# sunnyHelen/JPerceiver

Hardware: AMD Instinct MI355X
Metric: train images/sec (full train step, synthetic 3-frame batches) (higher is better)
Workload: dtype f32

## Files before the change

jperceiver_amd/csrc/conv_c16.hip:

```cpp
#include "jp_common.h"
#include <algorithm>

namespace {

constexpr int TPB = 256;

template <int CI, int CO, bool UPIN, bool SUMOUT, bool TRANS>
__global__ __launch_bounds__(TPB) void c16_conv_kernel(const float* __restrict__ x, const float* __restrict__ w,
                                                       const float* __restrict__ bias, float* __restrict__ y, int H, int W, int act,
                                                       int accumulate) {
    __shared__ __attribute__((aligned(16))) float wl[CI * 9 * CO];
    for (int i = threadIdx.x; i < CI * 9 * CO; i += TPB) {
        const int co = i % CO, tap = (i / CO) % 9, ci = i / (9 * CO);
        wl[i] = TRANS ? w[((size_t)ci * CO + co) * 9 + (8 - tap)] : w[((size_t)co * CI + ci) * 9 + tap];
    }
    __syncthreads();
    const int img = blockIdx.z;
    const int y0 = blockIdx.y * 32 + (threadIdx.x >> 4) * 2, x0 = blockIdx.x * 32 + (threadIdx.x & 15) * 2;
    const int sh = UPIN ? 1 : 0, hs = H >> sh, ws = W >> sh;
    const float* xp = x + (size_t)img * CI * hs * ws;
    int off[4][4];
#pragma unroll
    for (int a = 0; a < 4; ++a)
#pragma unroll
// ... 57 lines not shown
    }
}

constexpr int WG_R = 4, WG_C = 64;
template <int CI, int CO, bool UPIN, bool PART>
__global__ __launch_bounds__(TPB) void c16_wgrad_kernel(const float* __restrict__ x, const float* __restrict__ dy, float* __restrict__ dw,
                                                        int H, int W, int ntiles) {
    constexpr int P = CI * CO / TPB;
    static_assert(CI * CO % TPB == 0, "pairs per thread");
    constexpr int DP = WG_C + 1, XP = WG_C + 3;
    __shared__ float dT[CO * WG_R * DP];
    __shared__ float xT[CI * (WG_R + 2) * XP];
    const int sh = UPIN ? 1 : 0, hs = H >> sh, ws = W >> sh;
    const int tiles_x = W / WG_C, tiles_img = tiles_x * (H / WG_R);
    float acc[P][9];
#pragma unroll
    for (int k = 0; k < P; ++k)
#pragma unroll
        for (int t = 0; t < 9; ++t) acc[k][t] = 0.f;
    for (int T = blockIdx.x; T < ntiles; T += gridDim.x) {
        const int img = T / tiles_img, r_ = T - img * tiles_img;
        const int y0 = (r_ / tiles_x) * WG_R, x0 = (r_ % tiles_x) * WG_C;
        __syncthreads();
        const float* dp = dy + (size_t)img * CO * H * W;
        for (int i = threadIdx.x; i < CO * WG_R * WG_C; i += TPB) {
            const int c = i % WG_C, r = (i / WG_C) % WG_R, co = i / (WG_C * WG_R);
            dT[(co * WG_R + r) * DP + c] = dp[((size_t)co * H + y0 + r) * W + x0 + c];
        }
        const float* xp = x + (size_t)img * CI * hs * ws;
        for (int i = threadIdx.x; i < CI * (WG_R + 2) * (WG_C + 2); i += TPB) {
            const int c = i % (WG_C + 2), r = (i / (WG_C + 2)) % (WG_R + 2), ci = i / ((WG_C + 2) * (WG_R + 2));
            const int yy = y0 - 1 + r, xx = x0 - 1 + c;
            const bool in = (unsigned)yy < (unsigned)H && (unsigned)xx < (unsigned)W;
            xT[(ci * (WG_R + 2) + r) * XP + c] = in ? xp[((size_t)ci * hs + (yy >> sh)) * ws + (xx >> sh)] : 0.f;
        }
        __syncthreads();
#pragma unroll
        for (int k = 0; k < P; ++k) {
            const int q = threadIdx.x + TPB * k, co = q / CI, ci = q - co * CI;
            const float* dr = dT + co * WG_R * DP;
            const float* xr = xT + ci * (WG_R + 2) * XP;
#pragma unroll 1
            for (int r = 0; r < WG_R; ++r) {
                float w0[3], w1[3], w2[3];
#pragma unroll
                for (int t = 0; t < 3; ++t) {
                    w0[t] = xr[(r + t) * XP + 0];
                    w1[t] = xr[(r + t) * XP + 1];
                }
#pragma unroll 4
                for (int c = 0; c < WG_C; ++c) {
#pragma unroll
                    for (int t = 0; t < 3; ++t) w2[t] = xr[(r + t) * XP + c + 2];
                    const float d = dr[r * DP + c];
#pragma unroll
                    for (int t = 0; t < 3; ++t) {
                        acc[k][3 * t + 0] = fmaf(d, w0[t], acc[k][3 * t + 0]);
                        acc[k][3 * t + 1] = fmaf(d, w1[t], acc[k][3 * t + 1]);
                        acc[k][3 * t + 2] = fmaf(d, w2[t], acc[k][3 * t + 2]);
                    }
#pragma unroll
                    for (int t = 0; t < 3; ++t) { w0[t] = w1[t]; w1[t] = w2[t]; }
                }
            }
        }
    }
#pragma unroll
    for (int k = 0; k < P; ++k) {
        const int q = threadIdx.x + TPB * k;
#pragma unroll
        for (int t = 0; t < 9; ++t) {
            if (PART) dw[(size_t)blockIdx.x * (CO * CI * 9) + (size_t)q * 9 + t] = acc[k][t];
            else atomicAdd(dw + (size_t)q * 9 + t, acc[k][t]);
        }
    }
}

__global__ void c16_wgrad_fold_kernel(const float* __restrict__ part, float* __restrict__ dw, int n, int nblocks) {
    const int i = blockIdx.x * blockDim.x + threadIdx.x;
    if (i >= n) return;
    float s = 0.f;
    for (int b = 0; b < nblocks; ++b) s += part[(size_t)b * n + i];
    dw[i] += s;
}

template <bool UPIN, bool SUMOUT, bool TRANS>
int launch_conv(const float* x, const float* w, const float* bias, float* y, int N, int CI, int CO, int H, int W, int act, int accumulate,
                hipStream_t st) {
    const dim3 grid(W / 32, H / 32, N);
#define JP_GO(A, B)                                                                                                          \
    hipLaunchKernelGGL((c16_conv_kernel<A, B, UPIN, SUMOUT, TRANS>), grid, dim3(TPB), 0, st, x, w, bias, y, H, W, act, accumulate)
    if (CI == 16 && CO == 16) JP_GO(16, 16);
    else if (CI == 32 && CO == 32) JP_GO(32, 32);
    else if (CI == 32 && CO == 16) JP_GO(32, 16);
    else if (CI == 16 && CO == 32) JP_GO(16, 32);
    else return 1;
#undef JP_GO
    return 0;
}

}

bool jp_c16_ok(int Cin, int Cout, int KH, int stride, int pad, int pad_mode, int H, int W) {
    static const bool on = [] { const char* e = getenv("JP_C16"); return !(e && e[0] == '0'); }();
    return on && Cin == 16 && Cout == 16 && KH == 3 && stride == 1 && pad == 1 && pad_mode == 0 &&
           H % 32 == 0 && W % 64 == 0 && H >= 64;
}
int jp_c16_fwd(const float* x, int up, const float* w, const float* bias, float* y, int N, int Cin, int Cout, int H, int W, int act,
               hipStream_t st) {
    return up ? launch_conv<true, false, false>(x, w, bias, y, N, Cin, Cout, H, W, act, 0, st)
              : launch_conv<false, false, false>(x, w, bias, y, N, Cin, Cout, H, W, act, 0, st);
}
int jp_c16_dgrad(const float* dy, const float* w, float* dx, int up, int N, int Cin, int Cout, int H, int W, int accumulate,
                 hipStream_t st) {
    return up ? launch_conv<false, true, true>(dy, w, nullptr, dx, N, Cout, Cin, H, W, 0, accumulate, st)
              : launch_conv<false, false, true>(dy, w, nullptr, dx, N, Cout, Cin, H, W, 0, accumulate, st);
}
long jp_c16_wgrad_ws_floats(int N, int Cin, int Cout, int H, int W) {
    return (long)std::min(N * (H / WG_R) * (W / WG_C), 512) * Cout * Cin * 9;
}
int jp_c16_wgrad(const float* x, int up, const float* dy, float* dw, int N, int Cin, int Cout, int H, int W, hipStream_t st,
                 float* ws, long ws_floats) {
    const int ntiles = N * (H / WG_R) * (W / WG_C);
    const dim3 grid(std::min(ntiles, 512));
    const int nw = Cout * Cin * 9;
    const bool part = ws && ws_floats >= (long)grid.x * nw;
    float* out = part ? ws : dw;
#define JP_GO1(A, B, U, P) hipLaunchKernelGGL((c16_wgrad_kernel<A, B, U, P>), grid, dim3(TPB), 0, st, x, dy, out, H, W, ntiles)
#define JP_GO(A, B)                                                                     \
    {                                                                                   \
        if (up) { if (part) JP_GO1(A, B, true, true); else JP_GO1(A, B, true, false); } \
        else { if (part) JP_GO1(A, B, false, true); else JP_GO1(A, B, false, false); }  \
    }
    if (Cin == 16 && Cout == 16) JP_GO(16, 16)
    else if (Cin == 32 && Cout == 32) JP_GO(32, 32)
    else if (Cin == 32 && Cout == 16) JP_GO(32, 16)
    else if (Cin == 16 && Cout == 32) JP_GO(16, 32)
    else return 1;
#undef JP_GO
#undef JP_GO1
    if (part) hipLaunchKernelGGL(c16_wgrad_fold_kernel, dim3((nw + 255) / 256), dim3(256), 0, st, ws, dw, nw, (int)grid.x);
    return 0;
}
```

jperceiver_amd/csrc/conv_small.hip:

```cpp
#include "jp_common.h"
#include <algorithm>

namespace {

constexpr int TPB = 256;
constexpr int MAXCO = 4;

struct SrcSeg {
    const float* p;
    int C, sh;
};
struct Src3s {
    SrcSeg s[3];
    int nseg, H, W;
};

__device__ __forceinline__ void tap_offsets(int y, int x, int H, int W, int sh, int reflect, int off[9]) {
    const int w = W >> sh;
#pragma unroll
    for (int t = 0; t < 9; ++t) {
        int iy = y - 1 + t / 3, ix = x - 1 + t % 3;
        if (reflect) {
            iy = jp_reflect(iy, H);
            ix = jp_reflect(ix, W);
// ... 130 lines not shown
            }
            __syncthreads();
            const int xo = tx0 + tx;
            float g[4][CO];
#pragma unroll
            for (int j = 0; j < 4; ++j) {
                const int yo = ty0 + q * 4 + j;
                const bool ok = yo < H && xo < W;
#pragma unroll
                for (int c = 0; c < CO; ++c) g[j][c] = ok ? dp[(size_t)c * HW + yo * W + xo] : 0.f;
            }
#pragma unroll
            for (int r = 0; r < 6; ++r) {
                const float* row = tile + (q * 4 + r) * PW + tx;
                const float v0 = row[0], v1 = row[1], v2 = row[2];
#pragma unroll
                for (int j = 0; j < 4; ++j) {
                    const int ky = r - j;
                    if (ky < 0 || ky > 2) continue;
#pragma unroll
                    for (int c = 0; c < CO; ++c) {
                        acc[c * 9 + ky * 3 + 0] = fmaf(g[j][c], v0, acc[c * 9 + ky * 3 + 0]);
                        acc[c * 9 + ky * 3 + 1] = fmaf(g[j][c], v1, acc[c * 9 + ky * 3 + 1]);
                        acc[c * 9 + ky * 3 + 2] = fmaf(g[j][c], v2, acc[c * 9 + ky * 3 + 2]);
                    }
                }
            }
        }
    }
    const int lane = threadIdx.x & 63, wv = threadIdx.x >> 6;
#pragma unroll
    for (int i = 0; i < CO * 9; ++i) {
        const float s = jp_wave_sum(acc[i]);
        if (lane == 0) red[wv][i] = s;
    }
    __syncthreads();
    if (threadIdx.x < CO * 9) {
        const int i = threadIdx.x;
        const float s = red[0][i] + red[1][i] + red[2][i] + red[3][i];
        const int c = i / 9, t = i - c * 9;
        if (part) part[(((size_t)blockIdx.z * gridDim.x + blockIdx.x) * Cin + ci) * (CO * 9) + i] = s;
        else atomicAdd(dw + ((size_t)c * Cin + ci) * 9 + t, s);
    }
}

__global__ void conv_small_wgrad_fold_kernel(const float* __restrict__ part, float* __restrict__ dw, int Cin, int CO, int nwg) {
    const int i = blockIdx.x * blockDim.x + threadIdx.x;
    if (i >= Cin * CO * 9) return;
    const int ci = i / (CO * 9), r = i - ci * (CO * 9), c = r / 9, t = r - c * 9;
    float s = 0.f;
    for (int b = 0; b < nwg; ++b) s += part[((size_t)b * Cin + ci) * (CO * 9) + r];
    dw[((size_t)c * Cin + ci) * 9 + t] += s;
}

Src3s make_src(const float* x0, int c0, int up0, const float* x1, int c1, int up1, const float* x2, int c2, int up2,
               int H, int W) {
    Src3s s;
    s.nseg = 0;
    s.H = H; s.W = W;
    const float* ps[3] = {x0, x1, x2};
    const int cs[3] = {c0, c1, c2}, us[3] = {up0, up1, up2};
    for (int i = 0; i < 3; ++i)
        if (cs[i] > 0) { s.s[s.nseg].p = ps[i]; s.s[s.nseg].C = cs[i]; s.s[s.nseg].sh = us[i]; ++s.nseg; }
    for (int i = s.nseg; i < 3; ++i) s.s[i] = s.s[0];
    return s;
}

__device__ __forceinline__ void up_tap_range(int a, int r, int& lo, int& hi) {
    lo = a ? (r ? 2 : 0) : (r ? 1 : 0);
    hi = a ? (r ? 2 : 1) : (r ? 2 : 0);
}
__device__ __forceinline__ void up_build_weights(const float* __restrict__ w, float* wq, int C) {
    for (int i = threadIdx.x; i < 16 * C; i += blockDim.x) {
        const int c = i % C, q = i / C;
        int y0, y1, x0, x1;
        up_tap_range(q >> 3, (q >> 1) & 1, y0, y1);
        up_tap_range((q >> 2) & 1, q & 1, x0, x1);
        float v = 0.f;
        for (int dy = y0; dy <= y1; ++dy)
            for (int dx = x0; dx <= x1; ++dx) v += w[c * 9 + dy * 3 + dx];
        wq[i] = v;
    }
}
__device__ __forceinline__ void up_gather_D(const float* __restrict__ dyp, int i, int j, int h, int w, float D[16]) {
    const int W = 2 * w;
#pragma unroll
    for (int q = 0; q < 16; ++q) {
        const int a = q >> 3, b = (q >> 2) & 1, r = (q >> 1) & 1, s = q & 1;
        const int ri = i + 1 - a - r, rj = j + 1 - b - s;
        const int ei = (i == 0 && a == 0 && r == 0) ? 0 : ((i == h - 1 && a == 1 && r == 1) ? h - 1 : -1);
        const int ej = (j == 0 && b == 0 && s == 0) ? 0 : ((j == w - 1 && b == 1 && s == 1) ? w - 1 : -1);
        const bool rv = (unsigned)ri < (unsigned)h, cv = (unsigned)rj < (unsigned)w;
        float v = 0.f;
        if (rv && cv) v += dyp[(2 * ri + a) * W + 2 * rj + b];
        if (ei >= 0 && cv) v += dyp[(2 * ei + a) * W + 2 * rj + b];
        if (rv && ej >= 0) v += dyp[(2 * ri + a) * W + 2 * ej + b];
        if (ei >= 0 && ej >= 0) v += dyp[(2 * ei + a) * W + 2 * ej + b];
        D[q] = v;
    }
}

__global__ __launch_bounds__(TPB) void up_head_fwd_kernel(const float* __restrict__ x, const float* __restrict__ w,
                                                          const float* __restrict__ bias, float* __restrict__ y, int C,
                                                          int h, int wd, int act) {
    extern __shared__ float wq[];
    up_build_weights(w, wq, C);
    __syncthreads();
    const int img = blockIdx.y, hw = h * wd;
    const int p = blockIdx.x * TPB + threadIdx.x;
    if (p >= hw) return;
    const int i = p / wd, j = p - i * wd;
    const int r0 = max(i - 1, 0) * wd, r1 = i * wd, r2 = min(i + 1, h - 1) * wd;
    const int c0 = max(j - 1, 0), c2 = min(j + 1, wd - 1);
    float o00 = 0.f, o01 = 0.f, o10 = 0.f, o11 = 0.f;
    const float* xp = x + (size_t)img * C * hw;
    for (int c = 0; c < C; ++c) {
        const float* q = xp + (size_t)c * hw;
        const float v00 = q[r0 + c0], v01 = q[r0 + j], v02 = q[r0 + c2];
        const float v10 = q[r1 + c0], v11 = q[r1 + j], v12 = q[r1 + c2];
        const float v20 = q[r2 + c0], v21 = q[r2 + j], v22 = q[r2 + c2];
        const float* wc = wq + c;
        o00 += wc[0 * C] * v00 + wc[1 * C] * v01 + wc[2 * C] * v10 + wc[3 * C] * v11;
        o01 += wc[4 * C] * v01 + wc[5 * C] * v02 + wc[6 * C] * v11 + wc[7 * C] * v12;
        o10 += wc[8 * C] * v10 + wc[9 * C] * v11 + wc[10 * C] * v20 + wc[11 * C] * v21;
        o11 += wc[12 * C] * v11 + wc[13 * C] * v12 + wc[14 * C] * v21 + wc[15 * C] * v22;
    }
    const float bv = bias ? bias[0] : 0.f;
    float* yo = y + (size_t)img * 4 * hw + (size_t)(2 * i) * (2 * wd) + 2 * j;
    *reinterpret_cast<float2*>(yo) = make_float2(jp_act(o00 + bv, act), jp_act(o01 + bv, act));
    *reinterpret_cast<float2*>(yo + 2 * wd) = make_float2(jp_act(o10 + bv, act), jp_act(o11 + bv, act));
}

__global__ __launch_bounds__(TPB) void up_head_fwd2_kernel(const float* __restrict__ x, const float* __restrict__ w,
                                                           const float* __restrict__ bias, float* __restrict__ y, int C,
                                                           int h, int wd, int act) {
    extern __shared__ float wq[];
    up_build_weights(w, wq, C);
    __syncthreads();
    const int img = blockIdx.y, hw = h * wd, w2 = wd >> 1;
    const int p = blockIdx.x * TPB + threadIdx.x;
    if (p >= h * w2) return;
    const int i = p / w2, j = 2 * (p - i * w2);
    const int r0 = max(i - 1, 0) * wd, r1 = i * wd, r2 = min(i + 1, h - 1) * wd;
    const int cl = max(j - 1, 0), cr = min(j + 2, wd - 1);
    float o[2][4];
#pragma unroll
    for (int k = 0; k < 2; ++k)
#pragma unroll
        for (int q = 0; q < 4; ++q) o[k][q] = 0.f;
    const float* xp = x + (size_t)img * C * hw;
#pragma unroll 4
    for (int c = 0; c < C; ++c) {
        const float* q = xp + (size_t)c * hw;
        float v[3][4];
        const int rr[3] = {r0, r1, r2};
#pragma unroll
        for (int r = 0; r < 3; ++r) {
            const float2 m = *reinterpret_cast<const float2*>(q + rr[r] + j);
            v[r][0] = q[rr[r] + cl]; v[r][1] = m.x; v[r][2] = m.y; v[r][3] = q[rr[r] + cr];
        }
        float wc[16];
#pragma unroll
        for (int t = 0; t < 16; ++t) wc[t] = wq[t * C + c];
#pragma unroll
        for (int k = 0; k < 2; ++k) {
            o[k][0] += wc[0] * v[0][k] + wc[1] * v[0][k + 1] + wc[2] * v[1][k] + wc[3] * v[1][k + 1];
            o[k][1] += wc[4] * v[0][k + 1] + wc[5] * v[0][k + 2] + wc[6] * v[1][k + 1] + wc[7] * v[1][k + 2];
            o[k][2] += wc[8] * v[1][k] + wc[9] * v[1][k + 1] + wc[10] * v[2][k] + wc[11] * v[2][k + 1];
            o[k][3] += wc[12] * v[1][k + 1] + wc[13] * v[1][k + 2] + wc[14] * v[2][k + 1] + wc[15] * v[2][k + 2];
        }
    }
    const float bv = bias ? bias[0] : 0.f;
    float* yo = y + (size_t)img * 4 * hw + (size_t)(2 * i) * (2 * wd) + 2 * j;
    *reinterpret_cast<float4*>(yo) = make_float4(jp_act(o[0][0] + bv, act), jp_act(o[0][1] + bv, act), jp_act(o[1][0] + bv, act),
                                                 jp_act(o[1][1] + bv, act));
    *reinterpret_cast<float4*>(yo + 2 * wd) = make_float4(jp_act(o[0][2] + bv, act), jp_act(o[0][3] + bv, act),
                                                          jp_act(o[1][2] + bv, act), jp_act(o[1][3] + bv, act));
}

template <int groups>
__global__ __launch_bounds__(TPB) void up_head_fwd2s_kernel(const float* __restrict__ x, const float* __restrict__ w,
                                                           const float* __restrict__ bias, float* __restrict__ y, int C,
                                                           int h, int wd, int act) {
    extern __shared__ float wq[];
    __shared__ float red[3][64][8];
    up_build_weights(w, wq, C);
    __syncthreads();
    const int img = blockIdx.y, hw = h * wd, w2 = wd >> 1;
    constexpr int ppb = groups == 4 ? 64 : TPB;
    const int cg = threadIdx.x / ppb;
    const int p = blockIdx.x * ppb + (threadIdx.x % ppb);
    const bool live = p < h * w2;
    const int pc = live ? p : 0;
    const int i = pc / w2, j = 2 * (pc - i * w2);
    const int r0 = max(i - 1, 0) * wd, r1 = i * wd, r2 = min(i + 1, h - 1) * wd;
    const int cl = max(j - 1, 0), cr = min(j + 2, wd - 1);
    float o[2][4];
#pragma unroll
    for (int k = 0; k < 2; ++k)
#pragma unroll
        for (int q = 0; q < 4; ++q) o[k][q] = 0.f;
    const float* xp = x + (size_t)img * C * hw;
    const int cq = (C + groups - 1) / groups, cbeg = cg * cq, cend = min(C, cbeg + cq);
#pragma unroll 4
    for (int c = cbeg; c < cend; ++c) {
        const float* q = xp + (size_t)c * hw;
        float v[3][4];
        const int rr[3] = {r0, r1, r2};
#pragma unroll
        for (int r = 0; r < 3; ++r) {
            const float2 m = *reinterpret_cast<const float2*>(q + rr[r] + j);
            v[r][0] = q[rr[r] + cl]; v[r][1] = m.x; v[r][2] = m.y; v[r][3] = q[rr[r] + cr];
        }
        float wc[16];
#pragma unroll
        for (int t = 0; t < 16; ++t) wc[t] = wq[t * C + c];
#pragma unroll
        for (int k = 0; k < 2; ++k) {
            o[k][0] += wc[0] * v[0][k] + wc[1] * v[0][k + 1] + wc[2] * v[1][k] + wc[3] * v[1][k + 1];
            o[k][1] += wc[4] * v[0][k + 1] + wc[5] * v[0][k + 2] + wc[6] * v[1][k + 1] + wc[7] * v[1][k + 2];
            o[k][2] += wc[8] * v[1][k] + wc[9] * v[1][k + 1] + wc[10] * v[2][k] + wc[11] * v[2][k + 1];
            o[k][3] += wc[12] * v[1][k + 1] + wc[13] * v[1][k + 2] + wc[14] * v[2][k + 1] + wc[15] * v[2][k + 2];
        }
    }
    const int lp = threadIdx.x & 63;
    if (groups == 1) {
        if (!live) return;
    } else {
    if (cg > 0) {
#pragma unroll
        for (int k = 0; k < 8; ++k) red[cg - 1][lp][k] = o[k >> 2][k & 3];
    }
    __syncthreads();
    if (cg > 0 || !live) return;
#pragma unroll
    for (int g = 0; g < 3; ++g)
#pragma unroll
        for (int k = 0; k < 8; ++k) o[k >> 2][k & 3] += red[g][lp][k];
    }
    const float bv = bias ? bias[0] : 0.f;
    float* yo = y + (size_t)img * 4 * hw + (size_t)(2 * i) * (2 * wd) + 2 * j;
    *reinterpret_cast<float4*>(yo) = make_float4(jp_act(o[0][0] + bv, act), jp_act(o[0][1] + bv, act), jp_act(o[1][0] + bv, act),
                                                 jp_act(o[1][1] + bv, act));
    *reinterpret_cast<float4*>(yo + 2 * wd) = make_float4(jp_act(o[0][2] + bv, act), jp_act(o[0][3] + bv, act),
                                                          jp_act(o[1][2] + bv, act), jp_act(o[1][3] + bv, act));
}

__global__ __launch_bounds__(TPB) void up_head_dgrad_kernel(const float* __restrict__ dy, const float* __restrict__ w,
                                                            float* __restrict__ dx, int C, int h, int wd,
                                                            int accumulate) {
    extern __shared__ float wq[];
    up_build_weights(w, wq, C);
    __syncthreads();
    const int img = blockIdx.y, hw = h * wd;
    const int p = blockIdx.x * TPB + threadIdx.x;
    if (p >= hw) return;
    float D[16];
    up_gather_D(dy + (size_t)img * 4 * hw, p / wd, p % wd, h, wd, D);
    float* dp = dx + (size_t)img * C * hw + p;
    int c = 0;
    for (; c + 4 <= C; c += 4) {
        float old[4], v[4];
#pragma unroll
        for (int k = 0; k < 4; ++k) old[k] = accumulate ? dp[(size_t)(c + k) * hw] : 0.f;
#pragma unroll
        for (int k = 0; k < 4; ++k) {
            v[k] = 0.f;
#pragma unroll
            for (int q = 0; q < 16; ++q) v[k] = fmaf(wq[q * C + c + k], D[q], v[k]);
// ... 41 lines not shown
    if (threadIdx.x < UP_CB * 16) {
        const int k = threadIdx.x >> 4, q = threadIdx.x & 15;
        if (c0 + k < C) {
            const float s = red[0][threadIdx.x] + red[1][threadIdx.x] + red[2][threadIdx.x] + red[3][threadIdx.x];
            int y0, y1, x0, x1;
            up_tap_range(q >> 3, (q >> 1) & 1, y0, y1);
            up_tap_range((q >> 2) & 1, q & 1, x0, x1);
            for (int ty = y0; ty <= y1; ++ty)
                for (int tx = x0; tx <= x1; ++tx) atomicAdd(dw + (size_t)(c0 + k) * 9 + ty * 3 + tx, s);
        }
    }
}

__global__ __launch_bounds__(TPB) void up_head_D_kernel(const float* __restrict__ dy, float* __restrict__ D, int h, int wd) {
    const int img = blockIdx.y, hw = h * wd;
    const int p = blockIdx.x * TPB + threadIdx.x;
    if (p >= hw) return;
    float d[16];
    up_gather_D(dy + (size_t)img * 4 * hw, p / wd, p % wd, h, wd, d);
#pragma unroll
    for (int q = 0; q < 16; ++q) D[((size_t)img * 16 + q) * hw + p] = d[q];
}
constexpr int UPD_CB = 8;
__global__ __launch_bounds__(TPB) void up_head_wgrad_D_kernel(const float* __restrict__ x, const float* __restrict__ D,
                                                              float* __restrict__ dw, int C, int hw, int band,
                                                              float* __restrict__ part) {
    __shared__ float red[4][UPD_CB * 16];
    const int c0 = blockIdx.x * UPD_CB, img = blockIdx.z;
    const float* xp = x + ((size_t)img * C + c0) * hw;
    const float* dp = D + (size_t)img * 16 * hw;
    float acc[UPD_CB * 16];
#pragma unroll
    for (int i = 0; i < UPD_CB * 16; ++i) acc[i] = 0.f;
    const int pend = min(hw, (int)(blockIdx.y + 1) * band);
    for (int p = blockIdx.y * band + threadIdx.x; p < pend; p += TPB) {
        float d[16];
#pragma unroll
        for (int q = 0; q < 16; ++q) d[q] = dp[(size_t)q * hw + p];
#pragma unroll
        for (int k = 0; k < UPD_CB; ++k) {
            const float xv = (c0 + k < C) ? xp[(size_t)k * hw + p] : 0.f;
#pragma unroll
            for (int q = 0; q < 16; ++q) acc[k * 16 + q] = fmaf(xv, d[q], acc[k * 16 + q]);
        }
    }
    const int lane = threadIdx.x & 63, wv = threadIdx.x >> 6;
#pragma unroll
    for (int i = 0; i < UPD_CB * 16; ++i) {
        const float s = jp_wave_sum(acc[i]);
        if (lane == 0) red[wv][i] = s;
    }
    __syncthreads();
    if (threadIdx.x < UPD_CB * 16) {
        const int k = threadIdx.x >> 4, q = threadIdx.x & 15;
        if (c0 + k < C) {
            const float s = red[0][threadIdx.x] + red[1][threadIdx.x] + red[2][threadIdx.x] + red[3][threadIdx.x];
            if (part) {
                part[(((size_t)blockIdx.z * gridDim.y + blockIdx.y) * C + c0 + k) * 16 + q] = s;
            } else {
                int y0, y1, x0, x1;
                up_tap_range(q >> 3, (q >> 1) & 1, y0, y1);
                up_tap_range((q >> 2) & 1, q & 1, x0, x1);
                for (int ty = y0; ty <= y1; ++ty)
                    for (int tx = x0; tx <= x1; ++tx) atomicAdd(dw + (size_t)(c0 + k) * 9 + ty * 3 + tx, s);
            }
        }
    }
}
__global__ void up_head_wgrad_fold_kernel(const float* __restrict__ part, float* __restrict__ dw, int C, int nblk) {
    const int i = blockIdx.x * blockDim.x + threadIdx.x;
    if (i >= C * 9) return;
    const int c = i / 9, t = i - c * 9, ty = t / 3, tx = t - ty * 3;
    float s = 0.f;
    for (int q = 0; q < 16; ++q) {
        int y0, y1, x0, x1;
        up_tap_range(q >> 3, (q >> 1) & 1, y0, y1);
        up_tap_range((q >> 2) & 1, q & 1, x0, x1);
        if (ty < y0 || ty > y1 || tx < x0 || tx > x1) continue;
        for (int b = 0; b < nblk; ++b) s += part[((size_t)b * C + c) * 16 + q];
    }
    dw[i] += s;
}

}

int jp_conv_small_fwd(const float* x0, int c0, int up0, const float* x1, int c1, int up1, const float* x2, int c2, int up2,
                      const float* w, const float* bias, float* y, int N, int H, int W, int Cout, int act, int reflect,
                      hipStream_t st, int accumulate) {
    const int Cin = c0 + c1 + c2;
    const Src3s src = make_src(x0, c0, up0, x1, c1, up1, x2, c2, up2, H, W);
    const dim3 grid(jp_cdiv(H * W, TPB), N);
    const size_t lds = sizeof(float) * (size_t)Cout * Cin * 9;
#define JP_GO(CO) hipLaunchKernelGGL((conv_small_fwd_kernel<CO>), grid, dim3(TPB), lds, st, src, w, bias, y, Cin, act, reflect, accumulate)
    switch (Cout) {
        case 1: JP_GO(1); break;
        case 2: JP_GO(2); break;
        case 3: JP_GO(3); break;
        default: JP_GO(4); break;
    }
#undef JP_GO
    return 0;
}

static void small_wgrad_grid(int Cin, int N, int H, int W, bool tiled, dim3* grid, int* chunk) {
    if (tiled) { *grid = dim3(jp_cdiv(H, 64), Cin, N); *chunk = 0; return; }
    int chunks = std::max(1, 2048 / std::max(1, Cin * N));
    chunks = std::min(chunks, std::max(1, H * W / 4096));
    *chunk = jp_cdiv(jp_cdiv(H * W, chunks), TPB) * TPB;
    *grid = dim3(jp_cdiv(H * W, *chunk), Cin, N);
}
long jp_conv_small_wgrad_ws_floats(int N, int Cin, int H, int W, int Cout, int single_full_res) {
    dim3 g;
    int chunk;
    small_wgrad_grid(Cin, N, H, W, single_full_res && H >= 2 && W >= 2, &g, &chunk);
    return (long)g.x * g.z * Cin * std::min(std::max(Cout, 1), 4) * 9;
}
int jp_conv_small_wgrad(const float* x0, int c0, int up0, const float* x1, int c1, int up1, const float* x2, int c2,
                        int up2, const float* dy, float* dw, int N, int H, int W, int Cout, int reflect,
                        hipStream_t st, float* ws, long ws_floats) {
    const int Cin = c0 + c1 + c2;
    const Src3s src = make_src(x0, c0, up0, x1, c1, up1, x2, c2, up2, H, W);
    const bool tiled = src.nseg == 1 && src.s[0].sh == 0 && H >= 2 && W >= 2;
    const int CO = Cout <= 3 ? std::max(Cout, 1) : 4;
    dim3 grid;
    int chunk;
    small_wgrad_grid(Cin, N, H, W, tiled, &grid, &chunk);
    float* part = (ws && ws_floats >= (long)grid.x * grid.z * Cin * CO * 9) ? ws : nullptr;
    if (tiled) {
#define JP_GT(COv) hipLaunchKernelGGL((conv_small_wgrad_tiled_kernel<COv>), grid, dim3(TPB), 0, st, src.s[0].p, dy, dw, Cin, H, W, reflect, part)
        switch (Cout) {
            case 1: JP_GT(1); break;
            case 2: JP_GT(2); break;
            case 3: JP_GT(3); break;
            default: JP_GT(4); break;
        }
#undef JP_GT
    } else {
#define JP_GO(COv) hipLaunchKernelGGL((conv_small_wgrad_kernel<COv>), grid, dim3(TPB), 0, st, src, dy, dw, Cin, chunk, reflect, part)
        switch (Cout) {
            case 1: JP_GO(1); break;
            case 2: JP_GO(2); break;
            case 3: JP_GO(3); break;
            default: JP_GO(4); break;
        }
#undef JP_GO
    }
    if (part) hipLaunchKernelGGL(conv_small_wgrad_fold_kernel, dim3(jp_cdiv(Cin * CO * 9, 256)), dim3(256), 0, st, part, dw, Cin, CO,
                                 (int)(grid.x * grid.z));
    return 0;
}

int jp_up_head_fwd(const float* x, const float* w, const float* bias, float* y, int N, int C, int h, int wd, int act,
                   hipStream_t st) {
    if (wd % 4 == 0) {
        if ((long)N * h * (wd / 2) <= 8L * 2048)
            hipLaunchKernelGGL(up_head_fwd2s_kernel<4>, dim3(jp_cdiv(h * (wd / 2), 64), N), dim3(TPB), sizeof(float) * 16 * C, st, x, w,
                               bias, y, C, h, wd, act);
        else
            hipLaunchKernelGGL(up_head_fwd2_kernel, dim3(jp_cdiv(h * (wd / 2), TPB), N), dim3(TPB), sizeof(float) * 16 * C, st, x, w,
                               bias, y, C, h, wd, act);
        return 0;
    }
    hipLaunchKernelGGL(up_head_fwd_kernel, dim3(jp_cdiv(h * wd, TPB), N), dim3(TPB), sizeof(float) * 16 * C, st, x, w, bias, y,
                       C, h, wd, act);
    return 0;
}
int jp_up_head_dgrad(const float* dy, const float* w, float* dx, int N, int C, int h, int wd, int accumulate,
                     hipStream_t st) {
    hipLaunchKernelGGL(up_head_dgrad_kernel, dim3(jp_cdiv(h * wd, TPB), N), dim3(TPB), sizeof(float) * 16 * C, st, dy, w, dx, C,
                       h, wd, accumulate);
    return 0;
}
long jp_up_head_wgrad_ws_floats(int N, int C, int h, int wd) {
    const int hw = h * wd;
    const int bands = std::max(1, std::min(hw / (TPB * 16), 16));
    const int band = jp_cdiv(jp_cdiv(hw, bands), TPB) * TPB;
    return 16L * N * hw + 16L * C * jp_cdiv(hw, band) * N;
}
int jp_up_head_wgrad(const float* x, const float* dy, float* dw, int N, int C, int h, int wd, hipStream_t st, float* ws,
                     long ws_floats) {
    const int hw = h * wd;
    if (ws && ws_floats >= 16L * N * hw) {
        hipLaunchKernelGGL(up_head_D_kernel, dim3(jp_cdiv(hw, TPB), N), dim3(TPB), 0, st, dy, ws, h, wd);
        const int bands = std::max(1, std::min(hw / (TPB * 16), 16));
        const int band = jp_cdiv(jp_cdiv(hw, bands), TPB) * TPB;
        const int nb = jp_cdiv(hw, band);
        float* part = ws_floats >= 16L * N * hw + 16L * C * nb * N ? ws + 16L * N * hw : nullptr;
        hipLaunchKernelGGL(up_head_wgrad_D_kernel, dim3(jp_cdiv(C, UPD_CB), nb, N), dim3(TPB), 0, st, x, ws, dw, C, hw, band, part);
        if (part) hipLaunchKernelGGL(up_head_wgrad_fold_kernel, dim3(jp_cdiv(C * 9, 256)), dim3(256), 0, st, part, dw, C, nb * N);
        return 0;
    }
    const int bands = std::max(1, std::min(hw / (TPB * 16), 16));
    const int band = jp_cdiv(jp_cdiv(hw, bands), TPB) * TPB;
    hipLaunchKernelGGL(up_head_wgrad_kernel, dim3(jp_cdiv(C, UP_CB), jp_cdiv(hw, band), N), dim3(TPB), 0, st, x, dy, dw, C, h, wd,
                       band);
    return 0;
}
```

jperceiver_amd/csrc/jp_common.h:

```cpp
#pragma once
#include <hip/hip_runtime.h>
#include <stdint.h>

#define JP_OK 0
#define JP_EBADARG (-1)

extern "C" void jp_set_last_error(const char* msg);
void jp_prof_before(const char* tag, double flops, hipStream_t st);
void jp_prof_after(hipStream_t st);

#define JP_CHECK_ARG(cond, msg)                         \
    do {                                                \
        if (!(cond)) {                                  \
            jp_set_last_error(msg);                     \
            return JP_EBADARG;                          \
        }                                               \
    } while (0)

#define JP_LAUNCH_CHECK()                               \
    do {                                                \
        hipError_t e_ = hipGetLastError();              \
        if (e_ != hipSuccess) {                         \
            jp_set_last_error(hipGetErrorString(e_));   \
            return (int)e_;                             \
        }                                               \
        return JP_OK;                                   \
    } while (0)

#define JP_HIP(call)                                    \
    do {                                                \
        hipError_t e_ = (call);                         \
        if (e_ != hipSuccess) {                         \
            jp_set_last_error(hipGetErrorString(e_));   \
            return (int)e_;                             \
        }                                               \
    } while (0)

static inline int jp_cdiv(long a, long b) { return (int)((a + b - 1) / b); }

enum { JP_ACT_NONE = 0, JP_ACT_RELU = 1, JP_ACT_LEAKY = 2, JP_ACT_SIGMOID = 3 };
enum { JP_PAD_ZERO = 0, JP_PAD_REFLECT = 1 };

__device__ __forceinline__ float jp_act(float v, int act) {
    switch (act) {
        case JP_ACT_RELU: return v > 0.f ? v : 0.f;
        case JP_ACT_LEAKY: return v > 0.f ? v : 0.01f * v;
        case JP_ACT_SIGMOID: return 1.f / (1.f + __expf(-v));
        default: return v;
    }
}

__device__ __forceinline__ float jp_wave_sum(float v) {
#pragma unroll
    for (int o = 32; o > 0; o >>= 1) v += __shfl_xor(v, o, 64);
    return v;
}
__device__ __forceinline__ double jp_wave_sum_d(double v) {
#pragma unroll
    for (int o = 32; o > 0; o >>= 1) v += __shfl_xor(v, o, 64);
    return v;
}

__device__ __forceinline__ double jp_block_sum_d(double v, double* sm ) {
    v = jp_wave_sum_d(v);
    const int w = threadIdx.x >> 6;
    if ((threadIdx.x & 63) == 0) sm[w] = v;
    __syncthreads();
    double r = 0.0;
    if (threadIdx.x == 0) {
        const int nw = (blockDim.x + 63) >> 6;
        for (int i = 0; i < nw; ++i) r += sm[i];
    }
    __syncthreads();
    return r;
}

__host__ __device__ __forceinline__ unsigned jp_amag(unsigned bits) {
    const unsigned u = bits & 0x7fffffffu;
    return u >= (227u << 23) ? 0u : u;
}
__device__ __forceinline__ float jp_fmag(float v) {
    const float a = fabsf(v);
    return a < 0x1p100f ? a : 0.f;
}
constexpr int JP_AMAX_WAYS = 32, JP_AMAX_STRIDE = 16, JP_AMAX_SLOT = JP_AMAX_WAYS * JP_AMAX_STRIDE;
__device__ __forceinline__ unsigned jp_amax_way() {
    return ((blockIdx.x + 5u * blockIdx.y + 11u * blockIdx.z + (threadIdx.x >> 6)) & (JP_AMAX_WAYS - 1)) * JP_AMAX_STRIDE;
}
__device__ __forceinline__ float jp_slot_amax(const float* __restrict__ slot) {
    const int lane = threadIdx.x & 63;
    unsigned m = lane < JP_AMAX_WAYS ? __float_as_uint(slot[lane * JP_AMAX_STRIDE]) : 0u;
#pragma unroll
    for (int o = 32; o > 0; o >>= 1) m = max(m, (unsigned)__shfl_xor((int)m, o, 64));
    return __uint_as_float(m);
}
__device__ __forceinline__ void jp_wave_amax_commit(float mx, unsigned* out) {
    if (!out) return;
    unsigned m = jp_amag(__float_as_uint(mx));
#pragma unroll
    for (int o = 32; o > 0; o >>= 1) m = max(m, (unsigned)__shfl_xor((int)m, o, 64));
    if ((threadIdx.x & 63) == 0 && m) atomicMax(out + jp_amax_way(), m);
}
__device__ __forceinline__ void jp_block_amax_commit(float mx, unsigned* out) {
    if (!out) return;
    __shared__ unsigned jp_bam_[16];
    unsigned m = jp_amag(__float_as_uint(mx));
#pragma unroll
    for (int o = 32; o > 0; o >>= 1) m = max(m, (unsigned)__shfl_xor((int)m, o, 64));
    if ((threadIdx.x & 63) == 0) jp_bam_[threadIdx.x >> 6] = m;
    __syncthreads();
    if (threadIdx.x == 0) {
        const int nw = (blockDim.x + 63) >> 6;
        for (int i = 1; i < nw; ++i) m = max(m, jp_bam_[i]);
        if (m) atomicMax(out + jp_amax_way(), m);
    }
}
__device__ __forceinline__ int jp_reflect(int i, int n) {
    if (i < 0) i = -i;
    if (i >= n) i = 2 * n - 2 - i;
    return i;
}
```

Measured before the change: 127.1.

## Add tiled upsample-head forward, vectorized dgrad, direct wgrad and tree folds

Replaces the upsample-head forward with a shared-memory tiled kernel that stages input chunks and folded weights, double-buffered through registers. It adds a float4-vectorized dgrad, a direct wgrad that builds the 16 phase gradients on the fly instead of materializing a D buffer, and tree-style partial-sum fold kernels for both the upsample-head and c16 weight gradients. The old paths stay reachable through an env flag. This adds several complex kernels and risks register pressure and edge-case correctness in exchange for less memory traffic and better parallelism in the folds.

```diff
diff --git a/jperceiver_amd/csrc/conv_c16.hip b/jperceiver_amd/csrc/conv_c16.hip
--- a/jperceiver_amd/csrc/conv_c16.hip
+++ b/jperceiver_amd/csrc/conv_c16.hip
@@ -163,6 +163,13 @@
     float s = 0.f;
     for (int b = 0; b < nblocks; ++b) s += part[(size_t)b * n + i];
     dw[i] += s;
+}
+__global__ __launch_bounds__(TPB) void c16_wgrad_fold_tree_kernel(const float* __restrict__ part, float* __restrict__ dw, int n,
+                                                                  int nblocks) {
+    __shared__ float sh[TPB];
+    const int i = blockIdx.x * 16 + (threadIdx.x & 15);
+    const float s = jp_fold16(part + i, (size_t)n, nblocks, i < n, sh);
+    if (threadIdx.x < 16 && i < n) dw[i] += s;
 }
 
 template <bool UPIN, bool SUMOUT, bool TRANS>
@@ -220,6 +227,7 @@
     else return 1;
 #undef JP_GO
 #undef JP_GO1
-    if (part) hipLaunchKernelGGL(c16_wgrad_fold_kernel, dim3((nw + 255) / 256), dim3(256), 0, st, ws, dw, nw, (int)grid.x);
+    if (part && jp_up_head_v1()) hipLaunchKernelGGL(c16_wgrad_fold_kernel, dim3((nw + 255) / 256), dim3(256), 0, st, ws, dw, nw, (int)grid.x);
+    else if (part) hipLaunchKernelGGL(c16_wgrad_fold_tree_kernel, dim3((nw + 15) / 16), dim3(TPB), 0, st, ws, dw, nw, (int)grid.x);
     return 0;
 }
diff --git a/jperceiver_amd/csrc/conv_small.hip b/jperceiver_amd/csrc/conv_small.hip
--- a/jperceiver_amd/csrc/conv_small.hip
+++ b/jperceiver_amd/csrc/conv_small.hip
@@ -236,6 +236,26 @@
         wq[i] = v;
     }
 }
+__device__ __forceinline__ void up_build_weights_by_channel(const float* __restrict__ w, float* wq, int C) {
+    for (int c = threadIdx.x; c < C; c += blockDim.x) {
+        float t[9];
+#pragma unroll
+        for (int k = 0; k < 9; ++k) t[k] = w[c * 9 + k];
+#pragma unroll
+        for (int q = 0; q < 16; ++q) {
+            int y0, y1, x0, x1;
+            up_tap_range(q >> 3, (q >> 1) & 1, y0, y1);
+            up_tap_range((q >> 2) & 1, q & 1, x0, x1);
+            float v = 0.f;
+#pragma unroll
+            for (int dy = 0; dy < 3; ++dy)
+#pragma unroll
+                for (int dx = 0; dx < 3; ++dx)
+                    if (dy >= y0 && dy <= y1 && dx >= x0 && dx <= x1) v += t[dy * 3 + dx];
+            wq[q * C + c] = v;
+        }
+    }
+}
 __device__ __forceinline__ void up_gather_D(const float* __restrict__ dyp, int i, int j, int h, int w, float D[16]) {
     const int W = 2 * w;
 #pragma unroll
@@ -338,7 +358,7 @@
                                                            int h, int wd, int act) {
     extern __shared__ float wq[];
     __shared__ float red[3][64][8];
-    up_build_weights(w, wq, C);
+    up_build_weights_by_channel(w, wq, C);
     __syncthreads();
     const int img = blockIdx.y, hw = h * wd, w2 = wd >> 1;
     constexpr int ppb = groups == 4 ? 64 : TPB;
@@ -546,6 +566,377 @@
     dw[i] += s;
 }
 
+constexpr int UPT_W = 64, UPT_PITCH = 72;
+template <int PW, int CK>
+__global__ __launch_bounds__(TPB, PW == 2 ? 4 : 3) void up_head_fwd_tile_kernel(const float* __restrict__ x, const float* __restrict__ w,
+                                                               const float* __restrict__ bias, float* __restrict__ y, int C,
+                                                               int h, int wd, int act) {
+    constexpr int CG = 4 / PW, TR = 4 * PW, ROWS = TR + 2;
+    constexpr int NV = CK * ROWS * (UPT_W / 4);
+    constexpr int NVT = (NV + TPB - 1) / TPB;
+    constexpr int NR = CK * ROWS * 2;
+    constexpr int NRT = (NR + TPB - 1) / TPB;
+    constexpr int NWT = (CK * 16 + TPB - 1) / TPB;
+    constexpr int BUF = CK * ROWS * UPT_PITCH;
+    static_assert(CK % CG == 0, "channels of a chunk per wave group");
+    static_assert(BUF >= (CG - 1) * 16 * 64 * PW, "the partial sums reuse the tile buffer");
+    __shared__ __attribute__((aligned(16))) float tile[BUF];
+    __shared__ __attribute__((aligned(16))) float wq[CK * 16];
+    const int tid = threadIdx.x, lane = tid & 63, wv = tid >> 6;
+    const int pw = wv % PW, cg = wv / PW;
+    const int tiles_x = (wd + UPT_W - 1) / UPT_W;
+    const int x0 = (blockIdx.x % tiles_x) * UPT_W, y0 = (blockIdx.x / tiles_x) * TR;
+    const int img = blockIdx.y, hw = h * wd;
+    const int cols = min(UPT_W, wd - x0);
+    const float* xp = x + (size_t)img * C * hw;
+
+    int vsrc[NVT], rsrc[NRT];
+    const int vdst0 = (tid / (UPT_W / 4)) * UPT_PITCH + 4 + 4 * (tid % (UPT_W / 4));
+    const int rdst0 = (tid >> 1) * UPT_PITCH + ((tid & 1) ? 4 + cols : 3);
+#pragma unroll
+    for (int k = 0; k < NVT; ++k) {
+        const int i = tid + k * TPB;
+        const int c4 = i % (UPT_W / 4), r = (i / (UPT_W / 4)) % ROWS, cc = i / ((UPT_W / 4) * ROWS);
+        const int sy = min(max(y0 - 1 + r, 0), h - 1);
+        const bool ok = i < NV && 4 * c4 < cols;
+        vsrc[k] = ok ? cc * hw + sy * wd + x0 + 4 * c4 : -1;
+    }
+#pragma unroll
+    for (int k = 0; k < NRT; ++k) {
+        const int i = tid + k * TPB;
+        const int side = i & 1, r = (i >> 1) % ROWS, cc = (i >> 1) / ROWS;
+        const int sy = min(max(y0 - 1 + r, 0), h - 1);
+        const int sx = side ? min(x0 + cols, wd - 1) : max(x0 - 1, 0);
+        rsrc[k] = i < NR ? cc * hw + sy * wd + sx : -1;
+    }
+    int wsrc[NWT];
+    bool wx[NWT], wy[NWT];
+#pragma unroll
+    for (int k = 0; k < NWT; ++k) {
+        const int i = tid + k * TPB, q = i & 15;
+        int ty0, ty1, tx0, tx1;
+        up_tap_range(q >> 3, (q >> 1) & 1, ty0, ty1);
+        up_tap_range((q >> 2) & 1, q & 1, tx0, tx1);
+        wsrc[k] = i < CK * 16 ? (i >> 4) * 9 + ty0 * 3 + tx0 : -1;
+        wx[k] = tx1 > tx0; wy[k] = ty1 > ty0;
+    }
+    float4 vreg[NVT];
+    float rreg[NRT], wreg[NWT][4];
+#pragma unroll
+    for (int k = 0; k < NWT; ++k)
+#pragma unroll
+        for (int t = 0; t < 4; ++t) wreg[k][t] = 0.f;
+#pragma unroll
+    for (int k = 0; k < NVT; ++k) vreg[k] = make_float4(0.f, 0.f, 0.f, 0.f);
+#pragma unroll
+    for (int k = 0; k < NRT; ++k) rreg[k] = 0.f;
+    auto stage_load = [&](int c0) {
+        const float* xc = xp + (size_t)c0 * hw;
+        const int nch = min(CK, C - c0);
+#pragma unroll
+        for (int k = 0; k < NVT; ++k) {
+            const int i = tid + k * TPB;
+            if (vsrc[k] >= 0 && i / ((UPT_W / 4) * ROWS) < nch) vreg[k] = *reinterpret_cast<const float4*>(xc + vsrc[k]);
+        }
+#pragma unroll
+        for (int k = 0; k < NRT; ++k) {
+            const int i = tid + k * TPB;
+            if (rsrc[k] >= 0 && (i >> 1) / ROWS < nch) rreg[k] = xc[rsrc[k]];
+        }
+#pragma unroll
+        for (int k = 0; k < NWT; ++k) {
+            if (wsrc[k] >= 0 && (tid + k * TPB) >> 4 < nch) {
+                const float* wc = w + (size_t)c0 * 9 + wsrc[k];
+                wreg[k][0] = wc[0];
+                wreg[k][1] = wc[wx[k] ? 1 : 0];
+                wreg[k][2] = wc[wy[k] ? 3 : 0];
+                wreg[k][3] = wc[wx[k] && wy[k] ? 4 : 0];
+            }
+        }
+    };
+    auto stage_store = [&]() {
+        float* tb = tile;
+#pragma unroll
+        for (int k = 0; k < NVT; ++k)
+            if (vsrc[k] >= 0) *reinterpret_cast<float4*>(tb + vdst0 + k * (TPB / (UPT_W / 4)) * UPT_PITCH) = vreg[k];
+#pragma unroll
+        for (int k = 0; k < NRT; ++k)
+            if (rsrc[k] >= 0) tb[rdst0 + k * (TPB / 2) * UPT_PITCH] = rreg[k];
+#pragma unroll
+        for (int k = 0; k < NWT; ++k)
+            if (wsrc[k] >= 0) {
+                float v = 0.f + wreg[k][0];
+                if (wx[k]) v += wreg[k][1];
+                if (wy[k]) v += wreg[k][2];
+                if (wx[k] && wy[k]) v += wreg[k][3];
+                wq[tid + k * TPB] = v;
+            }
+    };
+
+    const int lr = 4 * pw + (lane >> 4), lc = 4 * (lane & 15);
+    float o[4][4];
+#pragma unroll
+    for (int k = 0; k < 4; ++k)
+#pragma unroll
+        for (int q = 0; q < 4; ++q) o[k][q] = 0.f;
+    const int nchunk = (C + CK - 1) / CK;
+    stage_load(0);
+    for (int ch = 0; ch < nchunk; ++ch) {
+        if (ch > 0) __syncthreads();
+        stage_store();
+        __syncthreads();
+        if (ch + 1 < nchunk) stage_load((ch + 1) * CK);
+        const int nch = min(CK, C - ch * CK);
+#pragma unroll
+        for (int k = 0; k < CK / CG; ++k) {
+            const int cc = cg * (CK / CG) + k;
+            if (cc < nch) {
+                const float* tp = tile + (cc * ROWS + lr) * UPT_PITCH + lc;
+                float v[3][6];
+#pragma unroll
+                for (int r = 0; r < 3; ++r) {
+                    const float4 l = *reinterpret_cast<const float4*>(tp + r * UPT_PITCH);
+                    const float4 m = *reinterpret_cast<const float4*>(tp + r * UPT_PITCH + 4);
+                    const float4 g = *reinterpret_cast<const float4*>(tp + r * UPT_PITCH + 8);
+                    v[r][0] = l.w;
+                    v[r][1] = m.x; v[r][2] = m.y; v[r][3] = m.z; v[r][4] = m.w;
+                    v[r][5] = g.x;
+                }
+                float wc[16];
+#pragma unroll
+                for (int t = 0; t < 4; ++t) {
+                    const float4 m = *reinterpret_cast<const float4*>(&wq[cc * 16 + 4 * t]);
+                    wc[4 * t] = m.x; wc[4 * t + 1] = m.y; wc[4 * t + 2] = m.z; wc[4 * t + 3] = m.w;
+                }
+#pragma unroll
+                for (int p = 0; p < 4; ++p)
+#pragma unroll
+                    for (int q = 0; q < 16; ++q) {
+                        const int a = q >> 3, b = (q >> 2) & 1, r = (q >> 1) & 1, s = q & 1;
+                        o[p][q >> 2] = fmaf(wc[q], v[a + r][p + b + s], o[p][q >> 2]);
+                    }
+            }
+        }
+    }
+    if (CG > 1) {
+        __syncthreads();
+        float* red = tile;
+        const int pt = pw * 64 + lane;
+        if (cg > 0) {
+#pragma unroll
+            for (int k = 0; k < 16; ++k) red[((cg - 1) * 16 + k) * (64 * PW) + pt] = o[k >> 2][k & 3];
+        }
+        __syncthreads();
+        if (cg > 0) return;
+#pragma unroll
+        for (int g = 0; g < CG - 1; ++g)
+#pragma unroll
+            for (int k = 0; k < 16; ++k) o[k >> 2][k & 3] += red[(g * 16 + k) * (64 * PW) + pt];
+    }
+    const int i = y0 + lr, j = x0 + lc;
+    if (i >= h || j >= wd) return;
+    const float bv = bias ? bias[0] : 0.f;
+    float* yo = y + (size_t)img * 4 * hw + (size_t)(2 * i) * (2 * wd) + 2 * j;
+#pragma unroll
+    for (int a = 0; a < 2; ++a) {
+        float* yr = yo + a * 2 * wd;
+        *reinterpret_cast<float4*>(yr) = make_float4(jp_act(o[0][2 * a] + bv, act), jp_act(o[0][2 * a + 1] + bv, act),
+                                                     jp_act(o[1][2 * a] + bv, act), jp_act(o[1][2 * a + 1] + bv, act));
+        *reinterpret_cast<float4*>(yr + 4) = make_float4(jp_act(o[2][2 * a] + bv, act), jp_act(o[2][2 * a + 1] + bv, act),
+                                                         jp_act(o[3][2 * a] + bv, act), jp_act(o[3][2 * a + 1] + bv, act));
+    }
+}
+
+__global__ __launch_bounds__(TPB) void up_head_dgrad4_kernel(const float* __restrict__ dy, const float* __restrict__ w,
+                                                             float* __restrict__ dx, int C, int h, int wd, int accumulate) {
+    extern __shared__ float wq[];
+    __shared__ __attribute__((aligned(16))) float Dl[16][TPB];
+    up_build_weights_by_channel(w, wq, C);
+    const int img = blockIdx.y, hw = h * wd;
+    const int pbase = blockIdx.x * TPB;
+    {
+        const int p = pbase + threadIdx.x;
+        float D[16];
+        if (p < hw) up_gather_D(dy + (size_t)img * 4 * hw, p / wd, p % wd, h, wd, D);
+        else {
+#pragma unroll
+            for (int q = 0; q < 16; ++q) D[q] = 0.f;
+        }
+#pragma unroll
+        for (int q = 0; q < 16; ++q) Dl[q][threadIdx.x] = D[q];
+    }
+    __syncthreads();
+    const int lane = threadIdx.x & 63, cg = threadIdx.x >> 6;
+    const int p4 = pbase + 4 * lane;
+    if (p4 >= hw) return;
+    float4 D[16];
+#pragma unroll
+    for (int q = 0; q < 16; ++q) D[q] = *reinterpret_cast<const float4*>(&Dl[q][4 * lane]);
+    const int cq = (C + 3) / 4, cbeg = cg * cq, cend = min(C, cbeg + cq);
+    float* dp = dx + (size_t)img * C * hw + p4;
+    int c = cbeg;
+    for (; c + 4 <= cend; c += 4) {
+        float4 old[4], v[4];
+#pragma unroll
+        for (int k = 0; k < 4; ++k)
+            old[k] = accumulate ? *reinterpret_cast<const float4*>(dp + (size_t)(c + k) * hw) : make_float4(0.f, 0.f, 0.f, 0.f);
+#pragma unroll
+        for (int k = 0; k < 4; ++k) {
+            v[k] = make_float4(0.f, 0.f, 0.f, 0.f);
+#pragma unroll
+            for (int q = 0; q < 16; ++q) {
+                const float wv = wq[q * C + c + k];
+                v[k].x = fmaf(wv, D[q].x, v[k].x); v[k].y = fmaf(wv, D[q].y, v[k].y);
+                v[k].z = fmaf(wv, D[q].z, v[k].z); v[k].w = fmaf(wv, D[q].w, v[k].w);
+            }
+        }
+#pragma unroll
+        for (int k = 0; k < 4; ++k)
+            *reinterpret_cast<float4*>(dp + (size_t)(c + k) * hw) =
+                make_float4(old[k].x + v[k].x, old[k].y + v[k].y, old[k].z + v[k].z, old[k].w + v[k].w);
+    }
+    for (; c < cend; ++c) {
+        float4 v = make_float4(0.f, 0.f, 0.f, 0.f);
+#pragma unroll
+        for (int q = 0; q < 16; ++q) {
+            const float wv = wq[q * C + c];
+            v.x = fmaf(wv, D[q].x, v.x); v.y = fmaf(wv, D[q].y, v.y); v.z = fmaf(wv, D[q].z, v.z); v.w = fmaf(wv, D[q].w, v.w);
+        }
+        float4* o = reinterpret_cast<float4*>(dp + (size_t)c * hw);
+        if (accumulate) { const float4 u = *o; v.x = u.x + v.x; v.y = u.y + v.y; v.z = u.z + v.z; v.w = u.w + v.w; }
+        *o = v;
+    }
+}
+
+__device__ __forceinline__ void up_patch_D(const float* __restrict__ dyp, int i, int j, int h, int w, float D[16]) {
+    const int W = 2 * w, H = 2 * h;
+    float P[4][4];
+#pragma unroll
+    for (int u = 0; u < 4; ++u) {
+        const int row = 2 * i - 1 + u;
+        const bool rv = (unsigned)row < (unsigned)H;
+        const float* rp = dyp + (size_t)min(max(row, 0), H - 1) * W + 2 * j;
+        const float2 m = *reinterpret_cast<const float2*>(rp);
+        const float l = rp[j > 0 ? -1 : 0], r = rp[j < w - 1 ? 2 : 1];
+        P[u][0] = (rv && j > 0) ? l : 0.f;
+        P[u][1] = rv ? m.x : 0.f;
+        P[u][2] = rv ? m.y : 0.f;
+        P[u][3] = (rv && j < w - 1) ? r : 0.f;
+    }
+#pragma unroll
+    for (int v = 0; v < 4; ++v) {
+        const float t = P[3][v] + P[1][v], bt = P[0][v] + P[2][v];
+        P[3][v] = i == 0 ? t : P[3][v];
+        P[0][v] = i == h - 1 ? bt : P[0][v];
+    }
+#pragma unroll
+    for (int u = 0; u < 4; ++u) {
+        const float t = P[u][3] + P[u][1], bt = P[u][0] + P[u][2];
+        P[u][3] = j == 0 ? t : P[u][3];
+        P[u][0] = j == w - 1 ? bt : P[u][0];
+    }
+#pragma unroll
+    for (int q = 0; q < 16; ++q) {
+        const int a = q >> 3, b = (q >> 2) & 1, r = (q >> 1) & 1, s = q & 1;
+        D[q] = P[3 - a - 2 * r][3 - b - 2 * s];
+    }
+}
+template <int M>
+__device__ __forceinline__ void up_wave_sums_step(float (&a)[UP_CB * 16], int lane) {
+    const bool hi = (lane & M) != 0;
+#pragma unroll
+    for (int k = 0; k < 2 * M; ++k) {
+        const float send = hi ? a[k] : a[k + 2 * M], keep = hi ? a[k + 2 * M] : a[k];
+        a[k] = keep + __shfl_xor(send, M, 64);
+    }
+}
+__device__ __forceinline__ void up_wave_sums128(float (&a)[UP_CB * 16], int lane) {
+    static_assert(UP_CB * 16 == 128, "two totals per lane");
+    up_wave_sums_step<32>(a, lane);
+    up_wave_sums_step<16>(a, lane);
+    up_wave_sums_step<8>(a, lane);
+    up_wave_sums_step<4>(a, lane);
+    up_wave_sums_step<2>(a, lane);
+    up_wave_sums_step<1>(a, lane);
+}
+__global__ __launch_bounds__(TPB) void up_head_wgrad_direct_kernel(const float* __restrict__ x, const float* __restrict__ dy,
+                                                                   float* __restrict__ part, int C, int h, int wd, int band) {
+    __shared__ float red[4][UP_CB * 16];
+    const int c0 = blockIdx.x * UP_CB, img = blockIdx.z, hw = h * wd;
+    const float* xp = x + ((size_t)img * C + c0) * hw;
+    const float* dyp = dy + (size_t)img * 4 * hw;
+    float acc[UP_CB * 16];
+#pragma unroll
+    for (int i = 0; i < UP_CB * 16; ++i) acc[i] = 0.f;
+    const int pend = min(hw, (int)(blockIdx.y + 1) * band);
+    float xq[3][UP_CB], Dn[16];
+    auto load_x = [&](int q, float (&xv)[UP_CB]) {
+#pragma unroll
+        for (int k = 0; k < UP_CB; ++k) xv[k] = (q < pend && c0 + k < C) ? xp[(size_t)k * hw + q] : 0.f;
+    };
+    int p = blockIdx.y * band + threadIdx.x;
+    load_x(p, xq[0]);
+    load_x(p + TPB, xq[1]);
+    load_x(p + 2 * TPB, xq[2]);
+    const int di = TPB / wd, dj = TPB % wd;
+    int i, j;
+    {
+        const int pc = min(p, hw - 1);
+        i = pc / wd; j = pc - i * wd;
+        up_patch_D(dyp, i, j, h, wd, Dn);
+    }
+    for (; p < pend; p += TPB) {
+        float xv[UP_CB], D[16];
+#pragma unroll
+        for (int k = 0; k < UP_CB; ++k) { xv[k] = xq[0][k]; xq[0][k] = xq[1][k]; xq[1][k] = xq[2][k]; }
+#pragma unroll
+        for (int q = 0; q < 16; ++q) D[q] = Dn[q];
+        load_x(p + 3 * TPB, xq[2]);
+        i += di; j += dj;
+        if (j >= wd) { j -= wd; ++i; }
+        if (p + TPB < pend) up_patch_D(dyp, i, j, h, wd, Dn);
+#pragma unroll
+        for (int k = 0; k < UP_CB; ++k)
+#pragma unroll
+            for (int q = 0; q < 16; ++q) acc[k * 16 + q] = fmaf(xv[k], D[q], acc[k * 16 + q]);
+    }
+    const int lane = threadIdx.x & 63, wv = threadIdx.x >> 6;
+    up_wave_sums128(acc, lane);
+    red[wv][2 * lane] = acc[0];
+    red[wv][2 * lane + 1] = acc[1];
+    __syncthreads();
+    if (threadIdx.x < UP_CB * 16) {
+        const int k = threadIdx.x >> 4, q = threadIdx.x & 15;
+        if (c0 + k < C)
+            part[(((size_t)blockIdx.z * gridDim.y + blockIdx.y) * C + c0 + k) * 16 + q] =
+                (red[0][threadIdx.x] + red[1][threadIdx.x]) + (red[2][threadIdx.x] + red[3][threadIdx.x]);
+    }
+}
+__global__ __launch_bounds__(TPB) void up_head_wgrad_fold_tree_kernel(const float* __restrict__ part, float* __restrict__ dw, int C,
+                                                                      int nblk) {
+    __shared__ float sh[TPB];
+    __shared__ float S[16];
+    const int c = blockIdx.x;
+    const float s = jp_fold16(part + (size_t)c * 16 + (threadIdx.x & 15), (size_t)C * 16, nblk, true, sh);
+    if (threadIdx.x < 16) S[threadIdx.x] = s;
+    __syncthreads();
+    if (threadIdx.x >= 9) return;
+    const int t = threadIdx.x, ty = t / 3, tx = t - ty * 3;
+    float v = 0.f;
+    for (int q = 0; q < 16; ++q) {
+        int y0, y1, x0, x1;
+        up_tap_range(q >> 3, (q >> 1) & 1, y0, y1);
+        up_tap_range((q >> 2) & 1, q & 1, x0, x1);
+        if (ty >= y0 && ty <= y1 && tx >= x0 && tx <= x1) v += S[q];
+    }
+    dw[c * 9 + t] += v;
+}
+
+}
+
+bool jp_up_head_v1() {
+    static const bool on = [] { const char* e = getenv("JP_UP_HEAD_V1"); return e && e[0] == '1'; }();
+    return on;
 }
 
 int jp_conv_small_fwd(const float* x0, int c0, int up0, const float* x1, int c1, int up1, const float* x2, int c2, int up2,
@@ -620,9 +1011,18 @@
         if ((long)N * h * (wd / 2) <= 8L * 2048)
             hipLaunchKernelGGL(up_head_fwd2s_kernel<4>, dim3(jp_cdiv(h * (wd / 2), 64), N), dim3(TPB), sizeof(float) * 16 * C, st, x, w,
                                bias, y, C, h, wd, act);
-        else
+        else if (jp_up_head_v1())
             hipLaunchKernelGGL(up_head_fwd2_kernel, dim3(jp_cdiv(h * (wd / 2), TPB), N), dim3(TPB), sizeof(float) * 16 * C, st, x, w,
                                bias, y, C, h, wd, act);
+        else {
+            const int tx = jp_cdiv(wd, UPT_W);
+            if ((long)N * jp_cdiv(h, 8) * tx >= 768)
+                hipLaunchKernelGGL((up_head_fwd_tile_kernel<2, 8>), dim3(jp_cdiv(h, 8) * tx, N), dim3(TPB), 0, st, x, w, bias, y, C, h,
+                                   wd, act);
+            else
+                hipLaunchKernelGGL((up_head_fwd_tile_kernel<1, 16>), dim3(jp_cdiv(h, 4) * tx, N), dim3(TPB), 0, st, x, w, bias, y, C, h,
+                                   wd, act);
+        }
         return 0;
     }
     hipLaunchKernelGGL(up_head_fwd_kernel, dim3(jp_cdiv(h * wd, TPB), N), dim3(TPB), sizeof(float) * 16 * C, st, x, w, bias, y,
@@ -631,12 +1031,21 @@
 }
 int jp_up_head_dgrad(const float* dy, const float* w, float* dx, int N, int C, int h, int wd, int accumulate,
                      hipStream_t st) {
-    hipLaunchKernelGGL(up_head_dgrad_kernel, dim3(jp_cdiv(h * wd, TPB), N), dim3(TPB), sizeof(float) * 16 * C, st, dy, w, dx, C,
-                       h, wd, accumulate);
+    if (!jp_up_head_v1() && (h * wd) % 4 == 0 && C <= 512)
+        hipLaunchKernelGGL(up_head_dgrad4_kernel, dim3(jp_cdiv(h * wd, TPB), N), dim3(TPB), sizeof(float) * 16 * C, st, dy, w, dx, C,
+                           h, wd, accumulate);
+    else
+        hipLaunchKernelGGL(up_head_dgrad_kernel, dim3(jp_cdiv(h * wd, TPB), N), dim3(TPB), sizeof(float) * 16 * C, st, dy, w, dx, C,
+                           h, wd, accumulate);
     return 0;
+}
+static int up_wgrad_band(int hw) {
+    const int bands = std::max(1, std::min(hw / (TPB * 32), 16));
+    return jp_cdiv(jp_cdiv(hw, bands), TPB) * TPB;
 }
 long jp_up_head_wgrad_ws_floats(int N, int C, int h, int wd) {
     const int hw = h * wd;
+    if (!jp_up_head_v1()) return 16L * C * jp_cdiv(hw, up_wgrad_band(hw)) * N;
     const int bands = std::max(1, std::min(hw / (TPB * 16), 16));
     const int band = jp_cdiv(jp_cdiv(hw, bands), TPB) * TPB;
     return 16L * N * hw + 16L * C * jp_cdiv(hw, band) * N;
@@ -644,7 +1053,14 @@
 int jp_up_head_wgrad(const float* x, const float* dy, float* dw, int N, int C, int h, int wd, hipStream_t st, float* ws,
                      long ws_floats) {
     const int hw = h * wd;
-    if (ws && ws_floats >= 16L * N * hw) {
+    if (!jp_up_head_v1()) {
+        const int band = up_wgrad_band(hw), nb = jp_cdiv(hw, band);
+        if (ws && ws_floats >= 16L * C * nb * N) {
+            hipLaunchKernelGGL(up_head_wgrad_direct_kernel, dim3(jp_cdiv(C, UP_CB), nb, N), dim3(TPB), 0, st, x, dy, ws, C, h, wd, band);
+            hipLaunchKernelGGL(up_head_wgrad_fold_tree_kernel, dim3(C), dim3(TPB), 0, st, ws, dw, C, nb * N);
+            return 0;
+        }
+    } else if (ws && ws_floats >= 16L * N * hw) {
         hipLaunchKernelGGL(up_head_D_kernel, dim3(jp_cdiv(hw, TPB), N), dim3(TPB), 0, st, dy, ws, h, wd);
         const int bands = std::max(1, std::min(hw / (TPB * 16), 16));
         const int band = jp_cdiv(jp_cdiv(hw, bands), TPB) * TPB;
diff --git a/jperceiver_amd/csrc/jp_common.h b/jperceiver_amd/csrc/jp_common.h
--- a/jperceiver_amd/csrc/jp_common.h
+++ b/jperceiver_amd/csrc/jp_common.h
@@ -75,6 +75,30 @@
     return r;
 }
 
+__device__ __forceinline__ float jp_fold16(const float* __restrict__ p, size_t stride, int nb, bool live, float* sh) {
+    const int s = threadIdx.x >> 4;
+    float a0 = 0.f, a1 = 0.f, a2 = 0.f, a3 = 0.f;
+    if (live) {
+        int b = s;
+        for (; b + 48 < nb; b += 64) {
+            a0 += p[(size_t)b * stride];
+            a1 += p[(size_t)(b + 16) * stride];
+            a2 += p[(size_t)(b + 32) * stride];
+            a3 += p[(size_t)(b + 48) * stride];
+        }
+        for (; b < nb; b += 16) a0 += p[(size_t)b * stride];
+    }
+    sh[threadIdx.x] = (a0 + a1) + (a2 + a3);
+    __syncthreads();
+#pragma unroll
+    for (int o = 8; o > 0; o >>= 1) {
+        if (s < o) sh[threadIdx.x] += sh[threadIdx.x + 16 * o];
+        __syncthreads();
+    }
+    return sh[threadIdx.x & 15];
+}
+bool jp_up_head_v1();
+
 __host__ __device__ __forceinline__ unsigned jp_amag(unsigned bits) {
     const unsigned u = bits & 0x7fffffffu;
     return u >= (227u << 23) ? 0u : u;
```

Result: no change. 126.8 (-0.2%).
